# hrnr/map-merge

Hardware: NVIDIA B200
Metric: pairwise_registrations_per_sec (higher is better)
Workload: dtype f32

## Files before the change

### map-merge_b200/csrc/knn_tc.cu

```cuda
#include <cuda.h>

#include <algorithm>
#include <cstring>

#include "mm3d_internal.cuh"

namespace mm3d {

namespace {

constexpr int TM = 128, TN = 128, TK = 32;
constexpr int A_TILES = 2;
constexpr int CTA_ROWS = A_TILES * TM;
constexpr int KB_BYTES = TM * TK * 4;
constexpr int A_RES_MAX_KB = 4;
constexpr int KMAXTC = 16;
constexpr int ACC_BUFS = 2;
constexpr int EPI_WARPS = 8;
constexpr int TC_THREADS = 64 + EPI_WARPS * 32;
constexpr int APAD = 36;
constexpr int EV_WARPS = 24;
constexpr int EV_LIST = 1024 + 32;
constexpr int EV_WORDS = 288;
constexpr int EV_BLOCKS_X = 16;
__host__ __device__ constexpr size_t ev_smem(int q) { return (size_t)EV_WARPS * (EV_LIST * 2 + EV_WORDS * 4 + (size_t)32 * q * 16); }
__host__ __device__ constexpr int tc_a_kb(int dreg, bool a_res) { return a_res ? (dreg > 0 ? 3 : A_RES_MAX_KB) : 0; }
__host__ __device__ constexpr int tc_stages(int dreg, bool a_res) { return a_res ? (dreg > 0 ? 6 : 5) : 3; }
__host__ __device__ constexpr size_t tc_smem(int dreg, bool a_res)
{
  return (size_t)A_TILES * tc_a_kb(dreg, a_res) * KB_BYTES + (size_t)tc_stages(dreg, a_res) * (a_res ? 1 : 1 + A_TILES) * KB_BYTES + 1024 + 256;
}

struct TcJob {
  int a_map, b_map;
  int na, nb;
  const float* normA;
  const float* origA;
  const float* origB;
  const float4* padA;
  const float4* padB;
  int k;
  int* idx;
  float* dist;
  float* audit;
  int* pick;
  float* thr;
  uint32_t* masks;
};

__device__ __forceinline__ uint32_t smem_u32(const void* p) { return (uint32_t)__cvta_generic_to_shared(p); }

__device__ __forceinline__ void mbar_init(uint64_t* bar, uint32_t count)
{
  asm volatile("mbarrier.init.shared::cta.b64 [%0], %1;" ::"r"(smem_u32(bar)), "r"(count));
}
__device__ __forceinline__ void mbar_wait(uint64_t* bar, uint32_t parity)
{
  asm volatile(
      "{\n\t"
      ".reg .pred p;\n\t"
      "WAIT_LOOP:\n\t"
      "mbarrier.try_wait.parity.shared::cta.b64 p, [%0], %1, %2;\n\t"
      "@p bra WAIT_DONE;\n\t"
      "bra WAIT_LOOP;\n\t"
      "WAIT_DONE:\n\t"
      "}\n" ::"r"(smem_u32(bar)),
      "r"(parity), "r"(20000u)
      : "memory");
}
__device__ __forceinline__ void mbar_arrive_expect_tx(uint64_t* bar, uint32_t bytes)
{
  asm volatile("mbarrier.arrive.expect_tx.shared::cta.b64 _, [%0], %1;" ::"r"(smem_u32(bar)), "r"(bytes) : "memory");
}
__device__ __forceinline__ void mbar_arrive(uint64_t* bar)
{
  asm volatile("mbarrier.arrive.shared::cta.b64 _, [%0];" ::"r"(smem_u32(bar)) : "memory");
}
__device__ __forceinline__ void tma_load_2d(const CUtensorMap* map, uint64_t* bar, void* dst, int c0, int c1)
{
  asm volatile("cp.async.bulk.tensor.2d.shared::cta.global.mbarrier::complete_tx::bytes [%0], [%1, {%3, %4}], [%2];" ::"r"(smem_u32(dst)),
               "l"((uint64_t)map), "r"(smem_u32(bar)), "r"(c0), "r"(c1)
               : "memory");
}
__device__ __forceinline__ void tc_fence_before() { asm volatile("tcgen05.fence::before_thread_sync;" ::: "memory"); }
__device__ __forceinline__ void tc_fence_after() { asm volatile("tcgen05.fence::after_thread_sync;" ::: "memory"); }
__device__ __forceinline__ void tc_commit(uint64_t* bar)
{
  asm volatile("tcgen05.commit.cta_group::1.mbarrier::arrive::one.shared::cluster.b64 [%0];" ::"r"(smem_u32(bar)) : "memory");
}
__device__ __forceinline__ void tc_mma_tf32(uint32_t tmem_d, uint64_t desc_a, uint64_t desc_b, uint32_t idesc, uint32_t accumulate)
{
  asm volatile(
      "{\n\t"
      ".reg .pred p;\n\t"
      "setp.ne.b32 p, %4, 0;\n\t"
      "tcgen05.mma.cta_group::1.kind::tf32 [%0], %1, %2, %3, p;\n\t"
      "}\n" ::"r"(tmem_d),
      "l"(desc_a), "l"(desc_b), "r"(idesc), "r"(accumulate)
      : "memory");
}
__device__ __forceinline__ uint64_t umma_desc_k_sw128(const void* tile)
{
  uint64_t d = 0;
  d |= (uint64_t)((smem_u32(tile) >> 4) & 0x3fff);
  d |= (uint64_t)1 << 16;
  d |= (uint64_t)(1024 >> 4) << 32;
  d |= (uint64_t)1 << 46;
  d |= (uint64_t)2 << 61;
  return d;
}
__device__ __forceinline__ void tmem_ld_32x32_issue(uint32_t taddr, uint32_t* r)
{
  asm volatile("tcgen05.ld.sync.aligned.32x32b.x32.b32 {%0, %1, %2, %3, %4, %5, %6, %7, %8, %9, %10, %11, %12, %13, %14, %15, %16, %17, %18, %19, %20, %21, %22, %23, %24, %25, %26, %27, %28, %29, %30, %31}, [%32];"
               : "=r"(r[0]), "=r"(r[1]), "=r"(r[2]), "=r"(r[3]), "=r"(r[4]), "=r"(r[5]), "=r"(r[6]), "=r"(r[7]), "=r"(r[8]), "=r"(r[9]), "=r"(r[10]), "=r"(r[11]), "=r"(r[12]), "=r"(r[13]), "=r"(r[14]), "=r"(r[15]), "=r"(r[16]), "=r"(r[17]), "=r"(r[18]), "=r"(r[19]), "=r"(r[20]), "=r"(r[21]), "=r"(r[22]), "=r"(r[23]), "=r"(r[24]), "=r"(r[25]), "=r"(r[26]), "=r"(r[27]), "=r"(r[28]), "=r"(r[29]), "=r"(r[30]), "=r"(r[31])
               : "r"(taddr));
}
__device__ __forceinline__ void tmem_ld_wait(uint32_t* r)
{
  asm volatile("tcgen05.wait::ld.sync.aligned;"
               : "+r"(r[0]), "+r"(r[1]), "+r"(r[2]), "+r"(r[3]), "+r"(r[4]), "+r"(r[5]), "+r"(r[6]), "+r"(r[7]), "+r"(r[8]), "+r"(r[9]), "+r"(r[10]), "+r"(r[11]), "+r"(r[12]), "+r"(r[13]), "+r"(r[14]), "+r"(r[15]), "+r"(r[16]), "+r"(r[17]), "+r"(r[18]), "+r"(r[19]), "+r"(r[20]), "+r"(r[21]), "+r"(r[22]), "+r"(r[23]), "+r"(r[24]), "+r"(r[25]), "+r"(r[26]), "+r"(r[27]), "+r"(r[28]), "+r"(r[29]), "+r"(r[30]), "+r"(r[31])
               :
               : "memory");
}

template <int THREADS>
__device__ __forceinline__ void named_bar_sync() { asm volatile("bar.sync 1, %0;" ::"n"(THREADS) : "memory"); }

__device__ __forceinline__ float fmin3(float a, float b, float c)
{
  float r;
  asm("min.f32 %0, %1, %2, %3;" : "=f"(r) : "f"(a), "f"(b), "f"(c));
  return r;
}

constexpr float TC_ERR_STORE = 3.1e-5f;

template <int KCAP>
__device__ __forceinline__ void topk_insert(float (&bd)[KCAP], int (&bi)[KCAP], float cd, int ci)
{
  bool shifting = false;
#pragma unroll
  for (int u = 0; u < KCAP; ++u) {
    if (shifting || cd < bd[u]) {
      const float td = bd[u];
      const int ti = bi[u];
      bd[u] = cd;
      bi[u] = ci;
      cd = td;
      ci = ti;
      shifting = true;
    }
  }
}

template <int DREG>
__device__ __forceinline__ float exact_dist(const TcJob& job, int D, int row, int col)
{
  float acc = 0.f;
  if constexpr (DREG > 0) {
    constexpr int Q = (DREG + 3) / 4;
    const float4* bp = job.padB + (size_t)col * Q;
    const float4* ap = job.padA + (size_t)row * Q;
    float a_[Q * 4], b_[Q * 4];
#pragma unroll
    for (int t = 0; t < Q; ++t) {
      const float4 v = __ldg(&bp[t]);
      b_[4 * t] = v.x; b_[4 * t + 1] = v.y; b_[4 * t + 2] = v.z; b_[4 * t + 3] = v.w;
      const float4 w = __ldg(&ap[t]);
      a_[4 * t] = w.x; a_[4 * t + 1] = w.y; a_[4 * t + 2] = w.z; a_[4 * t + 3] = w.w;
    }
#pragma unroll
    for (int t = 0; t < DREG; ++t) {
      const float diff = a_[t] - b_[t];
      acc += diff * diff;
    }
  } else {
    const float* a = job.origA + (size_t)row * D;
    const float* b = job.origB + (size_t)col * D;
    for (int t = 0; t < D; ++t) {
      const float diff = __ldg(&a[t]) - __ldg(&b[t]);
      acc += diff * diff;
    }
  }
  return acc;
}

template <int KCAP, int DREG, bool A_RES, bool AUDIT, int PASS>
__global__ void __launch_bounds__(TC_THREADS, 1) knn_tc_kernel(const TcJob* __restrict__ jobs, int job0, const CUtensorMap* __restrict__ mapsA,
                                                              const CUtensorMap* __restrict__ mapsB, int kblocks, int last_kb_half)
{
  constexpr int STAGES = tc_stages(DREG, A_RES);
  constexpr int STAGE_BYTES = (A_RES ? 1 : 1 + A_TILES) * KB_BYTES;
  constexpr int A_RES_BYTES = A_TILES * tc_a_kb(DREG, A_RES) * KB_BYTES;
  constexpr int ACC_COLS = A_TILES * TN;
  extern __shared__ uint8_t smem_raw[];
  uint8_t* a_res = smem_raw + ((1024u - (smem_u32(smem_raw) & 1023u)) & 1023u);
  uint8_t* tiles = a_res + A_RES_BYTES;
  uint64_t* full_bar = (uint64_t*)(tiles + (size_t)STAGES * STAGE_BYTES);
  uint64_t* empty_bar = full_bar + STAGES;
  uint64_t* tmem_full = empty_bar + STAGES;
  uint64_t* tmem_empty = tmem_full + ACC_BUFS;
  uint64_t* a_full = tmem_empty + ACC_BUFS;
  uint32_t* tmem_slot = (uint32_t*)(a_full + 1);

  const TcJob& job = jobs[job0 + blockIdx.y];
  const int na = job.na, nb = job.nb;
  const int m0 = blockIdx.x * CTA_ROWS;
  if (m0 >= na) return;
  const int warp = threadIdx.x >> 5, lane = threadIdx.x & 31;
  const int n_tiles = (nb + TN - 1) / TN;
  const int a_map = job.a_map, b_map = job.b_map;

  if (threadIdx.x == 0) {
    for (int s = 0; s < STAGES; ++s) {
      mbar_init(&full_bar[s], 1);
      mbar_init(&empty_bar[s], 1);
    }
    for (int b = 0; b < ACC_BUFS; ++b) {
      mbar_init(&tmem_full[b], 1);
      mbar_init(&tmem_empty[b], EPI_WARPS);
    }
    mbar_init(a_full, 1);
    asm volatile("fence.mbarrier_init.release.cluster;" ::: "memory");
  }
  if (warp == 1) {
    asm volatile("tcgen05.alloc.cta_group::1.sync.aligned.shared::cta.b32 [%0], %1;" ::"r"(smem_u32(tmem_slot)), "r"((uint32_t)(ACC_BUFS * ACC_COLS)) : "memory");
    asm volatile("tcgen05.relinquish_alloc_permit.cta_group::1.sync.aligned;" ::: "memory");
  }
  tc_fence_before();
  __syncthreads();
  tc_fence_after();
  const uint32_t tmem_base = *tmem_slot;

  if (warp == 0) {
    if (lane == 0) {
      if (A_RES) {
        mbar_arrive_expect_tx(a_full, (uint32_t)(A_TILES * kblocks) * KB_BYTES);
        for (int at = 0; at < A_TILES; ++at)
          for (int kb = 0; kb < kblocks; ++kb)
            tma_load_2d(&mapsA[a_map], a_full, a_res + (size_t)(at * tc_a_kb(DREG, A_RES) + kb) * KB_BYTES, kb * TK, m0 + at * TM);
      }
      int stage = 0;
      uint32_t phase = 0;
      for (int nt = 0; nt < n_tiles; ++nt)
        for (int kb = 0; kb < kblocks; ++kb) {
          mbar_wait(&empty_bar[stage], phase ^ 1);
          mbar_arrive_expect_tx(&full_bar[stage], STAGE_BYTES);
          uint8_t* st = tiles + (size_t)stage * STAGE_BYTES;
          tma_load_2d(&mapsB[b_map], &full_bar[stage], st, kb * TK, nt * TN);
          if (!A_RES)
            for (int at = 0; at < A_TILES; ++at) tma_load_2d(&mapsA[a_map], &full_bar[stage], st + (size_t)(1 + at) * KB_BYTES, kb * TK, m0 + at * TM);
          if (++stage == STAGES) { stage = 0; phase ^= 1; }
        }
    }
  } else if (warp == 1) {
    if (lane == 0) {
      const uint32_t idesc = (1u << 4) | (2u << 7) | (2u << 10) | ((uint32_t)(TN >> 3) << 17) | ((uint32_t)(TM >> 4) << 24);
      if (A_RES) {
        mbar_wait(a_full, 0);
        tc_fence_after();
      }
      int stage = 0;
      uint32_t phase = 0;
      for (int nt = 0; nt < n_tiles; ++nt) {
        const int buf = nt % ACC_BUFS;
        const uint32_t acc_phase = (uint32_t)(nt / ACC_BUFS) & 1u;
        mbar_wait(&tmem_empty[buf], acc_phase ^ 1);
        tc_fence_after();
        for (int kb = 0; kb < kblocks; ++kb) {
          mbar_wait(&full_bar[stage], phase);
          tc_fence_after();
          uint8_t* st = tiles + (size_t)stage * STAGE_BYTES;
          const uint64_t db = umma_desc_k_sw128(st);
          constexpr int PA[6] = {0, 2, 0, 1, 3, 1};
          constexpr int PB[6] = {0, 0, 2, 1, 1, 3};
          const int np = (last_kb_half && kb == kblocks - 1) ? 3 : 6;
#pragma unroll
          for (int at = 0; at < A_TILES; ++at) {
            const uint64_t da = umma_desc_k_sw128(A_RES ? a_res + (size_t)(at * tc_a_kb(DREG, A_RES) + kb) * KB_BYTES : st + (size_t)(1 + at) * KB_BYTES);
            const uint32_t tmem_d = tmem_base + (uint32_t)(buf * ACC_COLS + at * TN);
#pragma unroll
            for (int p = 0; p < 6; ++p)
              if (p < np) tc_mma_tf32(tmem_d, da + (uint64_t)(PA[p] * 2), db + (uint64_t)(PB[p] * 2), idesc, (kb | p) != 0 ? 1u : 0u);
          }
          tc_commit(&empty_bar[stage]);
          if (++stage == STAGES) { stage = 0; phase ^= 1; }
        }
        tc_commit(&tmem_full[buf]);
      }
    }
  } else {
    const int ew = warp - 2;
    const int q = warp & 3;
    const int at = ew >> 2;
    const int row = m0 + at * TM + q * 32 + lane;
    const bool live = row < na;
    const float INF = __int_as_float(0x7f800000);
    const uint32_t tmem_row = tmem_base + ((uint32_t)(q * 32) << 16) + (uint32_t)(at * TN);
    float t5[KCAP];
    int c5[KCAP];
#pragma unroll
    for (int i = 0; i < KCAP; ++i) {
      t5[i] = INF;
      c5[i] = -1;
    }
    uint32_t keep = 0xffffffe0u;
    asm volatile("" : "+r"(keep));
    float thr = -INF;
    uint32_t* mrow = nullptr;
    float* audit_row = nullptr;
    if constexpr (PASS == 1) {
      thr = live ? job.thr[row] : -INF;
      mrow = job.masks + (size_t)row * (size_t)(n_tiles * 4);
      if (AUDIT) audit_row = job.audit + (size_t)row * nb;
    }
    auto process = [&](uint32_t (&r)[32], int chunk_id) -> uint32_t {
      const int jbase = chunk_id * 32;
      const int left = nb - jbase;
      uint32_t msk = 0;
      if constexpr (PASS == 0) {
        if (left > 0) {
#pragma unroll
          for (int c = 0; c < 32; ++c) r[c] = (r[c] & keep) | (uint32_t)c;
          if (left < 32) {
#pragma unroll
            for (int c = 0; c < 32; ++c)
              if (c >= left) r[c] = 0x7f800000u;
          }
          float l1[11];
#pragma unroll
          for (int c = 0; c < 10; ++c) l1[c] = fmin3(__uint_as_float(r[3 * c]), __uint_as_float(r[3 * c + 1]), __uint_as_float(r[3 * c + 2]));
          l1[10] = fminf(__uint_as_float(r[30]), __uint_as_float(r[31]));
          const float l2a = fmin3(l1[0], l1[1], l1[2]), l2b = fmin3(l1[3], l1[4], l1[5]), l2c = fmin3(l1[6], l1[7], l1[8]);
          const float l2d = fminf(l1[9], l1[10]);
          const float m = fminf(fmin3(l2a, l2b, l2c), l2d);
          if (m < t5[KCAP - 1]) {
            float cd = m;
            int ci = chunk_id;
#pragma unroll
            for (int u = 0; u < KCAP; ++u) {
              if (cd < t5[u]) {
                const float td = t5[u];
                const int ti = c5[u];
                t5[u] = cd;
                c5[u] = ci;
                cd = td;
                ci = ti;
              }
            }
          }
        }
      } else {
        if (AUDIT) {
          if (live) {
#pragma unroll
            for (int c = 0; c < 32; ++c)
              if (c < left) audit_row[jbase + c] = __uint_as_float(r[c]);
          }
        }
        if (left > 0) {
          if (left < 32) {
#pragma unroll
            for (int c = 0; c < 32; ++c)
              if (c >= left) r[c] = 0x7f800000u;
          }
          float l1[11];
#pragma unroll
          for (int c = 0; c < 10; ++c) l1[c] = fmin3(__uint_as_float(r[3 * c]), __uint_as_float(r[3 * c + 1]), __uint_as_float(r[3 * c + 2]));
          l1[10] = fminf(__uint_as_float(r[30]), __uint_as_float(r[31]));
          const float l2a = fmin3(l1[0], l1[1], l1[2]), l2b = fmin3(l1[3], l1[4], l1[5]), l2c = fmin3(l1[6], l1[7], l1[8]);
          const float l2d = fminf(l1[9], l1[10]);
          const float m = fminf(fmin3(l2a, l2b, l2c), l2d);
          if (m <= thr) {
            uint32_t m0_ = 0, m1_ = 0, m2_ = 0, m3_ = 0;
#pragma unroll
            for (int c = 0; c < 8; ++c) {
              m0_ |= (__uint_as_float(r[c]) <= thr) ? (1u << c) : 0u;
              m1_ |= (__uint_as_float(r[8 + c]) <= thr) ? (1u << (8 + c)) : 0u;
              m2_ |= (__uint_as_float(r[16 + c]) <= thr) ? (1u << (16 + c)) : 0u;
              m3_ |= (__uint_as_float(r[24 + c]) <= thr) ? (1u << (24 + c)) : 0u;
            }
            msk = (m0_ | m1_) | (m2_ | m3_);
            if (left < 32) msk &= (1u << left) - 1u;
          }
        }
      }
      return msk;
    };
    uint32_t r0[32], r1[32];
    mbar_wait(&tmem_full[0], 0);
    tc_fence_after();
    tmem_ld_32x32_issue(tmem_row, r0);
    tmem_ld_wait(r0);
    for (int nt = 0; nt < n_tiles; ++nt) {
      const int buf = nt % ACC_BUFS;
      const uint32_t trow = tmem_row + (uint32_t)(buf * ACC_COLS);
      tmem_ld_32x32_issue(trow + 32, r1);
      const uint32_t k0 = process(r0, nt * 4);
      tmem_ld_wait(r1);
      tmem_ld_32x32_issue(trow + 64, r0);
      const uint32_t k1 = process(r1, nt * 4 + 1);
      tmem_ld_wait(r0);
      tmem_ld_32x32_issue(trow + 96, r1);
      const uint32_t k2 = process(r0, nt * 4 + 2);
      tmem_ld_wait(r1);
      tc_fence_before();
      __syncwarp();
      if (lane == 0) mbar_arrive(&tmem_empty[buf]);
      if (nt + 1 < n_tiles) {
        const int buf1 = (nt + 1) % ACC_BUFS;
        mbar_wait(&tmem_full[buf1], (uint32_t)((nt + 1) / ACC_BUFS) & 1u);
        tc_fence_after();
        tmem_ld_32x32_issue(tmem_row + (uint32_t)(buf1 * ACC_COLS), r0);
      }
      const uint32_t k3 = process(r1, nt * 4 + 3);
      if constexpr (PASS == 1) {
        if ((k0 | k1) | (k2 | k3)) *reinterpret_cast<uint4*>(mrow + nt * 4) = make_uint4(k0, k1, k2, k3);
      }
      if (nt + 1 < n_tiles) tmem_ld_wait(r0);
    }
    if constexpr (PASS == 0) {
      if (live) {
        int* pk = job.pick + (size_t)row * KCAP;
#pragma unroll
        for (int t = 0; t < KCAP; ++t) pk[t] = c5[t] >= 0 ? c5[t] * 32 + (int)(__float_as_uint(t5[t]) & 31u) : -1;
      }
    }
  }
  tc_fence_before();
  __syncthreads();
  if (warp == 1) {
    tc_fence_after();
    asm volatile("tcgen05.dealloc.cta_group::1.sync.aligned.b32 %0, %1;" ::"r"(tmem_base), "r"((uint32_t)(ACC_BUFS * ACC_COLS)) : "memory");
  }
}

template <int KCAP, int DREG>
__global__ void __launch_bounds__(128) knn_thr_kernel(const TcJob* __restrict__ jobs, int job0, int D)
{
  const TcJob& job = jobs[job0 + blockIdx.y];
  const int row = blockIdx.x * blockDim.x + threadIdx.x;
  if (row >= job.na) return;
  const float INF = __int_as_float(0x7f800000);
  const int k = min(job.k, KCAP);
  const int* pk = job.pick + (size_t)row * KCAP;
  float dmax = 0.f;
  bool all = true;
  for (int t = 0; t < k; ++t) {
    const int col = pk[t];
    if (col < 0) {
      all = false;
      break;
    }
    dmax = fmaxf(dmax, exact_dist<DREG>(job, D, row, col));
  }
  const float na_low = (1.0f - TC_ERR_STORE) * job.normA[row];
  job.thr[row] = all ? (dmax - na_low) + 1e-6f * (1.0f + fabsf(dmax) + na_low) : INF;
}

template <int KCAP, int DREG>
__global__ void __launch_bounds__(EV_WARPS * 32, 1) knn_eval_kernel(const TcJob* __restrict__ jobs, int job0, int D,
                                                                   unsigned long long* __restrict__ stats)
{
  constexpr int Q = DREG > 0 ? (DREG + 3) / 4 : 1;
  extern __shared__ float4 ev_smem_raw[];
  float4* stage_all = ev_smem_raw;
  uint32_t* words_all = (uint32_t*)(stage_all + (size_t)EV_WARPS * 32 * Q);
  unsigned short* list_all = (unsigned short*)(words_all + (size_t)EV_WARPS * EV_WORDS);
  const TcJob& job = jobs[job0 + blockIdx.y];
  const int na = job.na, nb = job.nb, k = job.k;
  const uint32_t* masks = job.masks;
  const float4* padA = job.padA;
  const float4* padB = job.padB;
  const int warp = threadIdx.x >> 5, lane = threadIdx.x & 31;
  const int n_chunks = ((nb + TN - 1) / TN) * 4;
  const float INF = __int_as_float(0x7f800000);
  const unsigned FULL = 0xffffffffu;
  unsigned short* lst = list_all + (size_t)warp * EV_LIST;
  uint32_t* wbuf = words_all + (size_t)warp * EV_WORDS;
  float4* stage = stage_all + (size_t)warp * 32 * Q;
  int gcand[Q], gpiece[Q];
#pragma unroll
  for (int i = 0; i < Q; ++i) {
    const int f = i * 32 + lane;
    gcand[i] = f / Q;
    gpiece[i] = f - gcand[i] * Q;
  }
  unsigned evals = 0, flushes = 0, rows_done = 0;
  const int rows_per_block = (na + (int)gridDim.x - 1) / (int)gridDim.x;
  const int row_end = min(na, ((int)blockIdx.x + 1) * rows_per_block);
  for (int row = (int)blockIdx.x * rows_per_block + warp; row < row_end; row += EV_WARPS) {
    float a_[Q * 4];
    if constexpr (DREG > 0) {
#pragma unroll
      for (int t = 0; t < Q; ++t) {
        const float4 w = __ldg(&padA[(size_t)row * Q + t]);
        a_[4 * t] = w.x; a_[4 * t + 1] = w.y; a_[4 * t + 2] = w.z; a_[4 * t + 3] = w.w;
      }
    }
    float bd[KCAP];
    int bi[KCAP];
#pragma unroll
    for (int t = 0; t < KCAP; ++t) {
      bd[t] = INF;
      bi[t] = -1;
    }
    auto step = [&](int base, int n) {
      const int jcol = lane < n ? (int)lst[base + lane] : 0;
      float d = INF;
      if constexpr (DREG > 0) {
        constexpr int H = (Q + 1) / 2;
#pragma unroll
        for (int h0 = 0; h0 < Q; h0 += H) {
          float4 v[H];
#pragma unroll
          for (int i = 0; i < H; ++i) {
            v[i] = make_float4(0.f, 0.f, 0.f, 0.f);
            if (h0 + i < Q && gcand[h0 + i] < n) v[i] = __ldg(&padB[(size_t)lst[base + gcand[h0 + i]] * Q + gpiece[h0 + i]]);
          }
#pragma unroll
          for (int i = 0; i < H; ++i)
            if (h0 + i < Q) stage[(h0 + i) * 32 + lane] = v[i];
        }
        __syncwarp();
        if (lane < n) {
          float acc = 0.f;
#pragma unroll
          for (int t = 0; t < Q; ++t) {
            const float4 bv = stage[lane * Q + t];
            const float b_[4] = {bv.x, bv.y, bv.z, bv.w};
#pragma unroll
            for (int u = 0; u < 4; ++u)
              if (4 * t + u < DREG) {
                const float diff = a_[4 * t + u] - b_[u];
                acc += diff * diff;
              }
          }
          d = acc;
        }
      } else {
        if (lane < n) d = exact_dist<DREG>(job, D, row, jcol);
      }
      unsigned better = __ballot_sync(FULL, d < bd[KCAP - 1]);
      while (better) {
        const int b = __ffs(better) - 1;
        const float dv = __shfl_sync(FULL, d, b);
        const int jv = __shfl_sync(FULL, jcol, b);
        topk_insert<KCAP>(bd, bi, dv, jv);
        better &= __ballot_sync(FULL, d < bd[KCAP - 1]) & ~((2u << b) - 1u);
      }
      evals += (unsigned)n;
      ++flushes;
      __syncwarp();
    };
    int pending = 0;
    const uint32_t* mp = masks + (size_t)row * n_chunks;
    for (int g0 = 0; g0 < n_chunks; g0 += EV_WORDS) {
      {
        uint32_t wv[EV_WORDS / 32];
#pragma unroll
        for (int u = 0; u < EV_WORDS / 32; ++u) {
          const int ch = g0 + u * 32 + lane;
          wv[u] = ch < n_chunks ? __ldcs(&mp[ch]) : 0u;
        }
#pragma unroll
        for (int u = 0; u < EV_WORDS / 32; ++u) wbuf[u * 32 + lane] = wv[u];
      }
      for (int g = 0; g < EV_WORDS && g0 + g < n_chunks; g += 32) {
        uint32_t w = wbuf[g + lane];
        if (!__any_sync(FULL, w != 0u)) continue;
        const int cnt = __popc(w);
        int pre = cnt;
#pragma unroll
        for (int o = 1; o < 32; o <<= 1) {
          const int t = __shfl_up_sync(FULL, pre, o);
          if (lane >= o) pre += t;
        }
        const int total = __shfl_sync(FULL, pre, 31);
        int pos = pending + pre - cnt;
        const int jb = (g0 + g + lane) * 32;
        while (w) {
          const int c = __ffs(w) - 1;
          w &= w - 1;
          lst[pos++] = (unsigned short)(jb + c);
        }
        __syncwarp();
        pending += total;
        int done = 0;
        while (pending - done >= 32) {
          step(done, 32);
          done += 32;
        }
        if (done > 0) {
          const int rest = pending - done;
          const unsigned short v = lane < rest ? lst[done + lane] : (unsigned short)0;
          __syncwarp();
          if (lane < rest) lst[lane] = v;
          __syncwarp();
          pending = rest;
        }
      }
    }
    if (pending > 0) step(0, pending);
    if (lane < k) {
      float dv = 0.f;
      int jv = -1;
#pragma unroll
      for (int u = 0; u < KCAP; ++u)
        if (u == lane && bi[u] >= 0) {
          dv = bd[u];
          jv = bi[u];
        }
      job.idx[(size_t)row * k + lane] = jv;
      job.dist[(size_t)row * k + lane] = dv;
    }
    ++rows_done;
  }
  if (stats && lane == 0 && rows_done) {
    atomicAdd(&stats[0], (unsigned long long)rows_done);
    atomicAdd(&stats[1], (unsigned long long)flushes);
    atomicAdd(&stats[2], (unsigned long long)evals);
  }
}

struct PrepJob {
  const float* src;
  float* formA;
  float* formB;
  float* norm;
  float* pad;
  int n;
};
constexpr int MEAN_CHUNKS = 32;
__global__ void __launch_bounds__(128) knn_tc_mean_partial_kernel(const PrepJob* __restrict__ jobs, int D, double* __restrict__ partial)
{
  const PrepJob& j = jobs[blockIdx.y];
  const int per = (j.n + MEAN_CHUNKS - 1) / MEAN_CHUNKS;
  const int r0 = blockIdx.x * per, r1 = min(j.n, r0 + per);
  for (int t = threadIdx.x; t < D; t += blockDim.x) {
    double s = 0.0;
    for (int r = r0; r < r1; ++r) s += (double)j.src[(size_t)r * D + t];
    partial[((size_t)blockIdx.y * MEAN_CHUNKS + blockIdx.x) * D + t] = s;
  }
}
__global__ void __launch_bounds__(128) knn_tc_mean_kernel(const double* __restrict__ partial, int n_partials, int D, double inv_rows,
                                                          float* __restrict__ mean)
{
  const int t = blockIdx.x * blockDim.x + threadIdx.x;
  if (t >= D) return;
  double s = 0.0;
  for (int p = 0; p < n_partials; ++p) s += partial[(size_t)p * D + t];
  mean[t] = (float)(s * inv_rows);
}

__device__ __forceinline__ float tf32_hi(float v) { return __uint_as_float(__float_as_uint(v) & 0xffffe000u); }

__global__ void __launch_bounds__(128) knn_tc_prep_kernel(const PrepJob* __restrict__ jobs, const float* __restrict__ mean, int D, int Kp,
                                                          int padw)
{
  const PrepJob& j = jobs[blockIdx.y];
  const int row = blockIdx.x;
  if (row >= j.n) return;
  const float* a = j.src + (size_t)row * D;
  float* fa = j.formA + (size_t)row * Kp;
  float* fb = j.formB + (size_t)row * Kp;
  __shared__ float s_norm;
  if (threadIdx.x == 0) {
    float s = 0.f;
    for (int t = 0; t < D; ++t) {
      const float v = a[t] - mean[t];
      s += v * v;
    }
    j.norm[row] = s;
    s_norm = s;
  }
  __syncthreads();
  const float nrm = (1.0f - TC_ERR_STORE) * s_norm;
  const float nh = tf32_hi(nrm), r1 = nrm - nh, nm = tf32_hi(r1), nl = r1 - nm;
  for (int t = threadIdx.x; t < Kp; t += blockDim.x) {
    const int kb = t >> 5, w = t & 31, is_lo = w >> 4, dim = kb * 16 + (w & 15);
    float va = 0.f, vb = 0.f;
    if (dim < D) {
      const float v = a[dim] - mean[dim];
      const float hi = tf32_hi(v);
      const float part = is_lo ? v - hi  : hi;
      va = -2.0f * part;
      vb = part;
    } else if (dim < D + 3 && !is_lo) {
      va = 1.0f;
      vb = dim == D ? nh : (dim == D + 1 ? nm : nl);
    }
    fa[t] = va;
    fb[t] = vb;
  }
  if (j.pad)
    for (int t = threadIdx.x; t < padw; t += blockDim.x) j.pad[(size_t)row * padw + t] = t < D ? a[t] : 0.f;
}

typedef CUresult (*EncodeTiledFn)(CUtensorMap*, CUtensorMapDataType, cuuint32_t, void*, const cuuint64_t*, const cuuint64_t*, const cuuint32_t*,
                                  const cuuint32_t*, CUtensorMapInterleave, CUtensorMapSwizzle, CUtensorMapL2promotion, CUtensorMapFloatOOBfill);

EncodeTiledFn encode_tiled()
{
  static EncodeTiledFn fn = nullptr;
  if (!fn) {
    void* p = nullptr;
    cudaDriverEntryPointQueryResult q;
    MM_CUDA(cudaGetDriverEntryPoint("cuTensorMapEncodeTiled", &p, cudaEnableDefault, &q));
    if (!p || q != cudaDriverEntryPointSuccess) throw CudaError("CUDA error: cuTensorMapEncodeTiled is not available");
    fn = (EncodeTiledFn)p;
  }
  return fn;
}

CUtensorMap make_map(float* base, int rows, int Kp)
{
  CUtensorMap m;
  memset(&m, 0, sizeof(m));
  const cuuint64_t dims[2] = {(cuuint64_t)Kp, (cuuint64_t)std::max(rows, 1)};
  const cuuint64_t strides[1] = {(cuuint64_t)Kp * 4};
  const cuuint32_t box[2] = {(cuuint32_t)TK, (cuuint32_t)TM};
  const cuuint32_t estr[2] = {1, 1};
  const CUresult r = encode_tiled()(&m, CU_TENSOR_MAP_DATA_TYPE_FLOAT32, 2, base, dims, strides, box, estr, CU_TENSOR_MAP_INTERLEAVE_NONE,
                                    CU_TENSOR_MAP_SWIZZLE_128B, CU_TENSOR_MAP_L2_PROMOTION_L2_128B, CU_TENSOR_MAP_FLOAT_OOB_FILL_NONE);
  if (r != CUDA_SUCCESS) throw CudaError("CUDA error: cuTensorMapEncodeTiled failed (" + std::to_string((int)r) + ")");
  return m;
}

}

void knn_tc_batch(Ctx& c, const std::vector<const float*>& desc, const std::vector<int>& n_rows, int D, const std::vector<KnnProblem>& probs,
                  KnnAudit* audit)
{
  if (probs.empty()) return;
  const int M = (int)desc.size();
  const int kblocks = (D + 3 + 15) / 16;
  const int last_kb_half = ((D + 3) - 16 * (kblocks - 1)) <= 8 ? 1 : 0;
  const int Kp = kblocks * TK;
  const bool reg_path = D == 33;
  const int padw = reg_path ? APAD : 0;
  std::vector<char> used(M, 0);
  for (const KnnProblem& p : probs) { used[p.a] = 1; used[p.b] = 1; }
  std::vector<DBuf<float>> formA(M), formB(M), norm(M), pad(M);
  std::vector<PrepJob> pj;
  int mxn = 0;
  for (int m = 0; m < M; ++m) {
    if (!used[m] || n_rows[m] == 0) continue;
    formA[m].alloc(c, (size_t)n_rows[m] * Kp);
    formB[m].alloc(c, (size_t)n_rows[m] * Kp);
    norm[m].alloc(c, n_rows[m]);
    if (reg_path) pad[m].alloc(c, (size_t)n_rows[m] * padw);
    pj.push_back(PrepJob{desc[m], formA[m].p, formB[m].p, norm[m].p, reg_path ? pad[m].p : nullptr, n_rows[m]});
    mxn = std::max(mxn, n_rows[m]);
  }
  if (pj.empty()) return;
  DBuf<PrepJob> dpj = to_device(c, pj);
  size_t rows_all = 0;
  for (const PrepJob& j : pj) rows_all += (size_t)j.n;
  DBuf<double> partial(c, pj.size() * MEAN_CHUNKS * (size_t)D);
  DBuf<float> mean(c, D);
  MM_LAUNCH(c, knn_tc_mean_partial_kernel, dim3(MEAN_CHUNKS, (unsigned)pj.size()), 128, 0, dpj.p, D, partial.p);
  MM_LAUNCH(c, knn_tc_mean_kernel, (D + 127) / 128, 128, 0, partial.p, (int)pj.size() * MEAN_CHUNKS, D, 1.0 / (double)rows_all, mean.p);
  MM_LAUNCH(c, knn_tc_prep_kernel, dim3(mxn, (unsigned)pj.size()), 128, 0, dpj.p, mean.p, D, Kp, padw);
  std::vector<CUtensorMap> hA(M), hB(M);
  for (int m = 0; m < M; ++m) {
    if (!used[m] || n_rows[m] == 0) {
      memset(&hA[m], 0, sizeof(CUtensorMap));
      memset(&hB[m], 0, sizeof(CUtensorMap));
      continue;
    }
    hA[m] = make_map(formA[m].p, n_rows[m], Kp);
    hB[m] = make_map(formB[m].p, n_rows[m], Kp);
  }
  DBuf<CUtensorMap> dA = to_device(c, hA), dB = to_device(c, hB);
  constexpr size_t MASK_WORDS_MAX = (size_t)3 << 27;
  struct Batch {
    int first, count, max_na;
    size_t words;
    double bytes;
  };
  std::vector<Batch> batches;
  std::vector<TcJob> tj;
  int kmax = 0;
  for (const KnnProblem& p : probs) kmax = std::max(kmax, p.k);
  const int kcap = kmax <= 5 ? 5 : (reg_path && kmax <= 10 ? 10 : KMAXTC);
  DBuf<float> audit_acc;
  size_t rows_total = 0;
  for (const KnnProblem& p : probs)
    if (p.na > 0 && n_rows[p.b] > 0) rows_total += (size_t)p.na;
  DBuf<float> thr(c, rows_total);
  DBuf<int> pick(c, rows_total * (size_t)kcap);
  size_t row_off = 0, words_max = 0;
  std::vector<size_t> mask_off;
  for (const KnnProblem& p : probs) {
    if (p.na == 0 || n_rows[p.b] == 0) continue;
    TcJob j;
    j.thr = thr.p + row_off;
    j.pick = pick.p + row_off * (size_t)kcap;
    row_off += (size_t)p.na;
    j.a_map = p.a;
    j.b_map = p.b;
    j.na = p.na;
    j.nb = n_rows[p.b];
    j.normA = norm[p.a].p;
    j.origA = desc[p.a];
    j.origB = desc[p.b];
    j.padA = reg_path ? (const float4*)pad[p.a].p : nullptr;
    j.padB = reg_path ? (const float4*)pad[p.b].p : nullptr;
    j.k = p.k;
    j.idx = p.idx;
    j.dist = p.dist;
    j.audit = nullptr;
    j.masks = nullptr;
    const size_t words = (size_t)j.na * (size_t)((j.nb + TN - 1) / TN * 4);
    if (batches.empty() || batches.back().words + words > MASK_WORDS_MAX || batches.back().count >= 65535)
      batches.push_back(Batch{(int)tj.size(), 0, 0, 0, 0.0});
    Batch& b = batches.back();
    mask_off.push_back(b.words);
    b.words += words;
    b.count += 1;
    b.max_na = std::max(b.max_na, j.na);
    b.bytes += 4.0 * D * ((double)j.na + j.nb) + 8.0 * j.k * j.na;
    words_max = std::max(words_max, b.words);
    tj.push_back(j);
  }
  if (tj.empty()) return;
  DBuf<uint32_t> masks(c, words_max);
  for (size_t t = 0; t < tj.size(); ++t) tj[t].masks = masks.p + mask_off[t];
  const bool do_audit = audit && tj.size() == 1 && reg_path && kmax <= 5;
  if (do_audit) {
    audit_acc.alloc(c, (size_t)tj[0].na * tj[0].nb);
    tj[0].audit = audit_acc.p;
  }
  DBuf<TcJob> dtj = to_device(c, tj);
  if (!c.knn_stats) {
    MM_CUDA(cudaMalloc((void**)&c.knn_stats, 3 * sizeof(unsigned long long)));
    MM_CUDA(cudaMemsetAsync(c.knn_stats, 0, 3 * sizeof(unsigned long long), c.stream));
  }
#define MM_TC(KCAP, DREG, RES, AUD)                                                                                                    \
  do {                                                                                                                                 \
    const size_t smem = tc_smem(DREG, RES);                                                                                            \
                                                      \
    MM_CUDA(cudaFuncSetAttribute(knn_tc_kernel<KCAP, DREG, RES, false, 0>, cudaFuncAttributeMaxDynamicSharedMemorySize, (int)smem));   \
    MM_CUDA(cudaFuncSetAttribute(knn_tc_kernel<KCAP, DREG, RES, AUD, 1>, cudaFuncAttributeMaxDynamicSharedMemorySize, (int)smem));     \
    const size_t esmem = ev_smem(DREG > 0 ? (DREG + 3) / 4 : 1);                                                                       \
    MM_CUDA(cudaFuncSetAttribute(knn_eval_kernel<KCAP, DREG>, cudaFuncAttributeMaxDynamicSharedMemorySize, (int)esmem));               \
    for (const Batch& b : batches) {                                                                                                   \
      const dim3 grid((b.max_na + CTA_ROWS - 1) / CTA_ROWS, (unsigned)b.count);                                                        \
      MM_CUDA(cudaMemsetAsync(masks.p, 0, b.words * sizeof(uint32_t), c.stream));                                                      \
      MM_BYTES(c, b.bytes);                                                                                                            \
      MM_LAUNCH(c, (knn_tc_kernel<KCAP, DREG, RES, false, 0>), grid, TC_THREADS, smem, dtj.p, b.first, dA.p, dB.p, kblocks,            \
                last_kb_half);                                                                                                         \
      MM_LAUNCH(c, (knn_thr_kernel<KCAP, DREG>), dim3((b.max_na + 127) / 128, (unsigned)b.count), 128, 0, dtj.p, b.first, D);          \
      MM_BYTES(c, b.bytes);                                                                                                            \
      MM_LAUNCH(c, (knn_tc_kernel<KCAP, DREG, RES, AUD, 1>), grid, TC_THREADS, smem, dtj.p, b.first, dA.p, dB.p, kblocks,              \
                last_kb_half);                                                                                                         \
      MM_BYTES(c, b.bytes);                                                                                                            \
      MM_LAUNCH(c, (knn_eval_kernel<KCAP, DREG>), dim3(EV_BLOCKS_X, (unsigned)b.count), EV_WARPS * 32, esmem, dtj.p, b.first, D,       \
                c.knn_stats);                                                                                                          \
    }                                                                                                                                  \
  } while (0)
  const bool res = kblocks <= A_RES_MAX_KB;
  if (do_audit) MM_TC(5, 33, true, true);
  else if (reg_path && kmax <= 5) MM_TC(5, 33, true, false);
  else if (reg_path && kmax <= 10) MM_TC(10, 33, true, false);
  else if (reg_path) MM_TC(KMAXTC, 33, true, false);
  else if (res && kmax <= 5) MM_TC(5, 0, true, false);
  else if (res) MM_TC(KMAXTC, 0, true, false);
  else if (kmax <= 5) MM_TC(5, 0, false, false);
  else MM_TC(KMAXTC, 0, false, false);
#undef MM_TC
  if (do_audit) {
    audit->acc.resize((size_t)tj[0].na * tj[0].nb);
    audit->norm_a.resize(tj[0].na);
    audit->norm_b.resize(tj[0].nb);
    audit_acc.download(c, audit->acc.data(), audit->acc.size());
    norm[probs[0].a].download(c, audit->norm_a.data(), audit->norm_a.size());
    norm[probs[0].b].download(c, audit->norm_b.data(), audit->norm_b.size());
    audit->err_store = TC_ERR_STORE;
    c.sync();
  }
}

}
```

Before: 1061.

## Share pass-1 distance tiles between symmetric A→B and B→A KNN problems

Detects adjacent KNN problems that are transposes of each other (A→B and B→A with the same k) and pairs them in a batch. Pass 0, threshold and eval still run over both directions. The pass-1 tensor-core GEMM runs only for one direction and also emits the transposed candidate masks for the mate problem, using warp ballots against the mate's per-column thresholds. This removes one of the two pass-1 distance-matrix computations per pair, at the cost of extra shuffles, ballots and scattered mask writes in the epilogue.

```diff
diff --git a/map-merge_b200/csrc/knn_tc.cu b/map-merge_b200/csrc/knn_tc.cu
--- a/map-merge_b200/csrc/knn_tc.cu
+++ b/map-merge_b200/csrc/knn_tc.cu
@@ -46,6 +46,7 @@
   int* pick;
   float* thr;
   uint32_t* masks;
+  int mate;
 };
 
 __device__ __forceinline__ uint32_t smem_u32(const void* p) { return (uint32_t)__cvta_generic_to_shared(p); }
@@ -185,7 +186,7 @@
   return acc;
 }
 
-template <int KCAP, int DREG, bool A_RES, bool AUDIT, int PASS>
+template <int KCAP, int DREG, bool A_RES, bool AUDIT, int PASS, bool PAIRED>
 __global__ void __launch_bounds__(TC_THREADS, 1) knn_tc_kernel(const TcJob* __restrict__ jobs, int job0, const CUtensorMap* __restrict__ mapsA,
                                                               const CUtensorMap* __restrict__ mapsB, int kblocks, int last_kb_half)
 {
@@ -314,7 +315,31 @@
       mrow = job.masks + (size_t)row * (size_t)(n_tiles * 4);
       if (AUDIT) audit_row = job.audit + (size_t)row * nb;
     }
-    auto process = [&](uint32_t (&r)[32], int chunk_id) -> uint32_t {
+    const unsigned FULL = 0xffffffffu;
+    const int rchunk = (m0 + at * TM + q * 32) >> 5;
+    const bool warp_live = rchunk * 32 < na;
+    float na_cmp = INF;
+    uint32_t live_rows = 0;
+    const TcJob* mate = nullptr;
+    if constexpr (PAIRED) {
+      mate = &jobs[job.mate];
+      if (live) {
+        const float na_low = (1.0f - TC_ERR_STORE) * job.normA[row];
+        na_cmp = na_low - 1e-6f * (1.0f + na_low);
+      }
+      live_rows = __ballot_sync(FULL, live);
+    }
+    float tcur[4] = {}, tnext[4] = {};
+    auto load_t = [&](float (&t)[4], int nt) {
+#pragma unroll
+      for (int u = 0; u < 4; ++u) {
+        const int j = (nt * 4 + u) * 32 + lane;
+        t[u] = j < nb ? __ldg(&mate->thr[j]) + (1.0f - TC_ERR_STORE) * __ldg(&mate->normA[j]) : -INF;
+      }
+    };
+    if constexpr (PAIRED && PASS == 1) load_t(tcur, 0);
+    auto fkey = [](float x) { const int i = __float_as_int(x); return i >= 0 ? i : i ^ 0x7fffffff; };
+    auto process = [&](uint32_t (&r)[32], int chunk_id, float tcol) -> uint32_t {
       const int jbase = chunk_id * 32;
       const int left = nb - jbase;
       uint32_t msk = 0;
@@ -383,6 +408,20 @@
             msk = (m0_ | m1_) | (m2_ | m3_);
             if (left < 32) msk &= (1u << left) - 1u;
           }
+          const uint32_t cols = PAIRED && warp_live ? __ballot_sync(FULL, fkey(tcol) >= __reduce_min_sync(FULL, fkey(m + na_cmp))) : 0u;
+          if (cols) {
+            uint32_t mine = 0;
+#pragma unroll
+            for (int c = 0; c < 32; ++c) {
+              if (cols & (1u << c)) {
+                const float tc = __shfl_sync(FULL, tcol, c);
+                const uint32_t b = __ballot_sync(FULL, __uint_as_float(r[c]) + na_cmp <= tc);
+                if (lane == c) mine = b;
+              }
+            }
+            mine &= live_rows;
+            if (mine) mate->masks[(size_t)(jbase + lane) * (size_t)(((na + TN - 1) / TN) * 4) + rchunk] = mine;
+          }
         }
       }
       return msk;
@@ -395,14 +434,17 @@
     for (int nt = 0; nt < n_tiles; ++nt) {
       const int buf = nt % ACC_BUFS;
       const uint32_t trow = tmem_row + (uint32_t)(buf * ACC_COLS);
+      if constexpr (PAIRED && PASS == 1) {
+        if (nt + 1 < n_tiles) load_t(tnext, nt + 1);
+      }
       tmem_ld_32x32_issue(trow + 32, r1);
-      const uint32_t k0 = process(r0, nt * 4);
+      const uint32_t k0 = process(r0, nt * 4, tcur[0]);
       tmem_ld_wait(r1);
       tmem_ld_32x32_issue(trow + 64, r0);
-      const uint32_t k1 = process(r1, nt * 4 + 1);
+      const uint32_t k1 = process(r1, nt * 4 + 1, tcur[1]);
       tmem_ld_wait(r0);
       tmem_ld_32x32_issue(trow + 96, r1);
-      const uint32_t k2 = process(r0, nt * 4 + 2);
+      const uint32_t k2 = process(r0, nt * 4 + 2, tcur[2]);
       tmem_ld_wait(r1);
       tc_fence_before();
       __syncwarp();
@@ -413,9 +455,13 @@
         tc_fence_after();
         tmem_ld_32x32_issue(tmem_row + (uint32_t)(buf1 * ACC_COLS), r0);
       }
-      const uint32_t k3 = process(r1, nt * 4 + 3);
+      const uint32_t k3 = process(r1, nt * 4 + 3, tcur[3]);
       if constexpr (PASS == 1) {
         if ((k0 | k1) | (k2 | k3)) *reinterpret_cast<uint4*>(mrow + nt * 4) = make_uint4(k0, k1, k2, k3);
+      }
+      if constexpr (PAIRED && PASS == 1) {
+#pragma unroll
+        for (int u = 0; u < 4; ++u) tcur[u] = tnext[u];
       }
       if (nt + 1 < n_tiles) tmem_ld_wait(r0);
     }
@@ -775,7 +821,8 @@
   DBuf<CUtensorMap> dA = to_device(c, hA), dB = to_device(c, hB);
   constexpr size_t MASK_WORDS_MAX = (size_t)3 << 27;
   struct Batch {
-    int first, count, max_na;
+    int first, count, max_na, max_nb;
+    bool paired;
     size_t words;
     double bytes;
   };
@@ -791,9 +838,7 @@
   DBuf<float> thr(c, rows_total);
   DBuf<int> pick(c, rows_total * (size_t)kcap);
   size_t row_off = 0, words_max = 0;
-  std::vector<size_t> mask_off;
-  for (const KnnProblem& p : probs) {
-    if (p.na == 0 || n_rows[p.b] == 0) continue;
+  auto make_job = [&](const KnnProblem& p) {
     TcJob j;
     j.thr = thr.p + row_off;
     j.pick = pick.p + row_off * (size_t)kcap;
@@ -812,18 +857,59 @@
     j.dist = p.dist;
     j.audit = nullptr;
     j.masks = nullptr;
-    const size_t words = (size_t)j.na * (size_t)((j.nb + TN - 1) / TN * 4);
-    if (batches.empty() || batches.back().words + words > MASK_WORDS_MAX || batches.back().count >= 65535)
-      batches.push_back(Batch{(int)tj.size(), 0, 0, 0, 0.0});
+    j.mate = -1;
+    return j;
+  };
+  auto words_of = [](const TcJob& j) { return (size_t)j.na * (size_t)((j.nb + TN - 1) / TN * 4); };
+  auto bytes_of = [&](const TcJob& j) { return 4.0 * D * ((double)j.na + j.nb) + 8.0 * j.k * j.na; };
+  auto pairs_with = [&](const KnnProblem& p, const KnnProblem& q) {
+    return !audit && q.a == p.b && q.b == p.a && q.k == p.k && p.na == n_rows[p.a] && q.na == n_rows[q.a] && p.na >= p.k && q.na >= p.k;
+  };
+  std::vector<size_t> mask_off;
+  std::vector<TcJob> mates;
+  std::vector<size_t> mate_off;
+  auto close_pairs = [&]() {
+    if (batches.empty() || !batches.back().paired) return;
+    const int first = batches.back().first, count = batches.back().count;
+    for (int t = 0; t < count; ++t) tj[first + t].mate = first + count + t;
+    tj.insert(tj.end(), mates.begin(), mates.end());
+    mask_off.insert(mask_off.end(), mate_off.begin(), mate_off.end());
+    mates.clear();
+    mate_off.clear();
+  };
+  for (size_t t = 0; t < probs.size(); ++t) {
+    const KnnProblem& p = probs[t];
+    if (p.na == 0 || n_rows[p.b] == 0) continue;
+    const bool paired = t + 1 < probs.size() && pairs_with(p, probs[t + 1]);
+    TcJob j = make_job(p);
+    TcJob jm;
+    size_t words = words_of(j);
+    double bytes = bytes_of(j);
+    if (paired) {
+      jm = make_job(probs[++t]);
+      words += words_of(jm);
+      bytes += bytes_of(jm);
+    }
+    if (batches.empty() || batches.back().paired != paired || batches.back().words + words > MASK_WORDS_MAX ||
+        batches.back().count >= (paired ? 32767 : 65535)) {
+      close_pairs();
+      batches.push_back(Batch{(int)tj.size(), 0, 0, 0, paired, 0, 0.0});
+    }
     Batch& b = batches.back();
     mask_off.push_back(b.words);
+    if (paired) {
+      mate_off.push_back(b.words + words_of(j));
+      mates.push_back(jm);
+    }
     b.words += words;
     b.count += 1;
     b.max_na = std::max(b.max_na, j.na);
-    b.bytes += 4.0 * D * ((double)j.na + j.nb) + 8.0 * j.k * j.na;
+    b.max_nb = std::max(b.max_nb, j.nb);
+    b.bytes += bytes;
     words_max = std::max(words_max, b.words);
     tj.push_back(j);
   }
+  close_pairs();
   if (tj.empty()) return;
   DBuf<uint32_t> masks(c, words_max);
   for (size_t t = 0; t < tj.size(); ++t) tj[t].masks = masks.p + mask_off[t];
@@ -841,22 +927,29 @@
   do {                                                                                                                                 \
     const size_t smem = tc_smem(DREG, RES);                                                                                            \
                                                       \
-    MM_CUDA(cudaFuncSetAttribute(knn_tc_kernel<KCAP, DREG, RES, false, 0>, cudaFuncAttributeMaxDynamicSharedMemorySize, (int)smem));   \
-    MM_CUDA(cudaFuncSetAttribute(knn_tc_kernel<KCAP, DREG, RES, AUD, 1>, cudaFuncAttributeMaxDynamicSharedMemorySize, (int)smem));     \
+    MM_CUDA(cudaFuncSetAttribute(knn_tc_kernel<KCAP, DREG, RES, false, 0, false>, cudaFuncAttributeMaxDynamicSharedMemorySize, (int)smem)); \
+    MM_CUDA(cudaFuncSetAttribute(knn_tc_kernel<KCAP, DREG, RES, AUD, 1, false>, cudaFuncAttributeMaxDynamicSharedMemorySize, (int)smem));   \
+    MM_CUDA(cudaFuncSetAttribute(knn_tc_kernel<KCAP, DREG, RES, false, 1, true>, cudaFuncAttributeMaxDynamicSharedMemorySize, (int)smem));  \
     const size_t esmem = ev_smem(DREG > 0 ? (DREG + 3) / 4 : 1);                                                                       \
     MM_CUDA(cudaFuncSetAttribute(knn_eval_kernel<KCAP, DREG>, cudaFuncAttributeMaxDynamicSharedMemorySize, (int)esmem));               \
     for (const Batch& b : batches) {                                                                                                   \
-      const dim3 grid((b.max_na + CTA_ROWS - 1) / CTA_ROWS, (unsigned)b.count);                                                        \
+      const int n_dir = b.paired ? 2 * b.count : b.count;                       \
+      const int rows_max = b.paired ? std::max(b.max_na, b.max_nb) : b.max_na;                                                         \
+      const dim3 grid0((rows_max + CTA_ROWS - 1) / CTA_ROWS, (unsigned)n_dir), grid((b.max_na + CTA_ROWS - 1) / CTA_ROWS, (unsigned)b.count);\
       MM_CUDA(cudaMemsetAsync(masks.p, 0, b.words * sizeof(uint32_t), c.stream));                                                      \
       MM_BYTES(c, b.bytes);                                                                                                            \
-      MM_LAUNCH(c, (knn_tc_kernel<KCAP, DREG, RES, false, 0>), grid, TC_THREADS, smem, dtj.p, b.first, dA.p, dB.p, kblocks,            \
+      MM_LAUNCH(c, (knn_tc_kernel<KCAP, DREG, RES, false, 0, false>), grid0, TC_THREADS, smem, dtj.p, b.first, dA.p, dB.p, kblocks,    \
                 last_kb_half);                                                                                                         \
-      MM_LAUNCH(c, (knn_thr_kernel<KCAP, DREG>), dim3((b.max_na + 127) / 128, (unsigned)b.count), 128, 0, dtj.p, b.first, D);          \
+      MM_LAUNCH(c, (knn_thr_kernel<KCAP, DREG>), dim3((rows_max + 127) / 128, (unsigned)n_dir), 128, 0, dtj.p, b.first, D);            \
       MM_BYTES(c, b.bytes);                                                                                                            \
-      MM_LAUNCH(c, (knn_tc_kernel<KCAP, DREG, RES, AUD, 1>), grid, TC_THREADS, smem, dtj.p, b.first, dA.p, dB.p, kblocks,              \
-                last_kb_half);                                                                                                         \
+      if (b.paired)                                                                                                                    \
+        MM_LAUNCH(c, (knn_tc_kernel<KCAP, DREG, RES, false, 1, true>), grid, TC_THREADS, smem, dtj.p, b.first, dA.p, dB.p, kblocks,    \
+                  last_kb_half);                                                                                                       \
+      else                                                                                                                             \
+        MM_LAUNCH(c, (knn_tc_kernel<KCAP, DREG, RES, AUD, 1, false>), grid, TC_THREADS, smem, dtj.p, b.first, dA.p, dB.p, kblocks,     \
+                  last_kb_half);                                                                                                       \
       MM_BYTES(c, b.bytes);                                                                                                            \
-      MM_LAUNCH(c, (knn_eval_kernel<KCAP, DREG>), dim3(EV_BLOCKS_X, (unsigned)b.count), EV_WARPS * 32, esmem, dtj.p, b.first, D,       \
+      MM_LAUNCH(c, (knn_eval_kernel<KCAP, DREG>), dim3(EV_BLOCKS_X, (unsigned)n_dir), EV_WARPS * 32, esmem, dtj.p, b.first, D,         \
                 c.knn_stats);                                                                                                          \
     }                                                                                                                                  \
   } while (0)
```

Measured after the change: 1024, median of 6. 3.5% lower.
